# google/deepvariant

Measured on AMD Instinct MI355X. Metric: candidate pileups/sec (encode+CNN), higher is better.
Workload: dtype u8 (encoder) / f16 MFMA, f32 accumulate (CNN); 1 GPU; configs[1] shape: synthetic 30x Illumina pileups, WGS 100x221x7, HIP encode + Inception-v3 MFMA on 1 MI355X per rank, random-init weights; parallelism=interval shards x1, all-gather of probs, collective_world_size=1

## Files before the change

deepvariant_amd/csrc/conv_mfma.h:

```cpp
#ifndef DV_CONV_MFMA_H_
#define DV_CONV_MFMA_H_

#include "conv_common.h"

namespace dv {
namespace convk {

constexpr int kSlabChunks = 8;

inline size_t resident_lds_bytes(const ConvArgs& a) {
  return static_cast<size_t>(a.n_slabs) * kSlabChunks * 3 * 32 * kChunk * 2;
}

void launch_conv(const ConvArgs& a, int nb, hipStream_t stream);
void launch_conv_resident(const ConvArgs& a, int n_cus, hipStream_t stream);
void launch_conv_pool_resident(const ConvArgs& a, int n_cus, hipStream_t stream);
void launch_conv_pool1x1(const ConvArgs& a, int nb, hipStream_t stream);

}
}

#endif
```

deepvariant_amd/csrc/conv_mfma.hip:

```cpp
#include <algorithm>
#include <cstdlib>
#include <type_traits>

#include "conv_mfma.h"

using namespace dv::convk;

namespace {

constexpr int prefetch_depth(int , int ) { return 4; }

struct ChunkWalk {
  int kh, kw;
  unsigned tap_off;
  unsigned chunk_off;
  __device__ __forceinline__ unsigned off() const { return chunk_off + tap_off; }
  __device__ __forceinline__ void advance(const ConvArgs& p) {
    const bool row_end = ++kw == p.KW;
    kw = row_end ? 0 : kw;
    tap_off += row_end ? static_cast<unsigned>((p.ig.wp - p.KW + 1) * 16) : 16u;
    kh += row_end ? 1 : 0;
    const bool taps_end = kh == p.KH;
    kh = taps_end ? 0 : kh;
    tap_off = taps_end ? 0u : tap_off;
// ... 314 lines not shown
  DV_STORE_SLAB(0)
  __syncthreads();

  const int frag_off = (lane >> 5) * (BN * 8) + (lane & 31) * 8;
  if (wave_blank) {
    const int n_full_b = p.n_chunks / SLAB;
    for (int s = 0; s < n_full_b; ++s) {
      const int next = s + 1 < (p.n_chunks + SLAB - 1) / SLAB ? s + 1 : s;
      DV_LOAD_SLAB(next)
      DV_STORE_SLAB((s + 1) & 1)
      __syncthreads();
    }
    copy_blank_wave<NB, PT>(p, n_tile, pn, poh, pow_, mvalid, lane);
    return;
  }
  SidePool<PT> side;
  auto k_loop = [&](auto split_tag, auto pool_tag, const int n_chunks) {
    constexpr bool S = decltype(split_tag)::value;
    constexpr bool P = decltype(pool_tag)::value;
    SidePool<PT>* const sp = P ? &side : nullptr;
    const int tile_slabs = (n_chunks + SLAB - 1) / SLAB;
#ifdef DV_ABLATE_LOOP
    const int n_full = n_chunks < 0 ? 1 : 0;
    const int rem = 0;
#else
    const int n_full = n_chunks / SLAB;
    const int rem = n_chunks - n_full * SLAB;
#endif
    for (int s = 0; s < n_full; ++s) {
      const int next = s + 1 < tile_slabs ? s + 1 : s;
      DV_LOAD_SLAB(next)
      if constexpr (WIDE) {
        conv_slab_wide<NB, PT, SLAB>(p, rsrc, smem + (s & 1) * SLAB_HALFS + frag_off, walk, base, xf, acc);
      } else {
        conv_slab<NB, PT, SLAB, 0, S, P>(p, rsrc, smem + (s & 1) * SLAB_HALFS + frag_off, walk, base, xf, acc, sp);
      }
      DV_STORE_SLAB((s + 1) & 1)
      __syncthreads();
    }
    if (rem) {
      const _Float16* wslab = smem + (n_full & 1) * SLAB_HALFS + frag_off;
      if constexpr (WIDE) {
        conv_slab_wide<NB, PT, 4>(p, rsrc, wslab, walk, base, xf, acc);
        if constexpr (SLAB > 4) {
          if (rem > 4) conv_slab_wide<NB, PT, 4>(p, rsrc, wslab + 4 * BN * kChunk, walk, base, xf, acc);
        }
      } else {
      conv_slab<NB, PT, 4, 0, S, P>(p, rsrc, wslab, walk, base, xf, acc, sp);
      if constexpr (SLAB > 4) {
        if (rem > 4) conv_slab<NB, PT, 4, 4, S, P>(p, rsrc, wslab + 4 * BN * kChunk, walk, base, xf, acc, sp);
      }
      }
    }
  };
  if constexpr (SPLIT) {
    if (n_tile < p.split_tiles) {
      k_loop(std::true_type{}, std::false_type{}, p.n_chunks);
    } else {
      k_loop(std::false_type{}, std::false_type{}, p.n_chunks >> 1);
    }
  } else if constexpr (SIDE_POOL) {
    side.tap = 0;
    side.cc = 0;
    side.cc_mod = 0;
    side.n_tiles = p.n_tiles;
    side.my_tile = n_tile;
    side.taps = p.KH * p.KW;
    side.n_cc = p.Cin / kChunk;
    side.gstride2 = 2u * static_cast<unsigned>(p.side_pool_og.hp * p.side_pool_og.wp);
    side.out = reinterpret_cast<uint4_t*>(p.side_pool_out);
#pragma unroll
    for (int pt = 0; pt < PT; ++pt) {
      const _Float16 lowest = static_cast<_Float16>(-65504.f);
      side.best[pt] = half8_t{lowest, lowest, lowest, lowest, lowest, lowest, lowest, lowest};
      side.ok[pt] = mvalid[pt];
      side.at[pt] = static_cast<unsigned>(
          ((pn[pt] * p.side_pool_og.groups + p.side_pool_goff + (lane >> 5)) * p.side_pool_og.hp + poh[pt] +
           p.side_pool_og.halo) * p.side_pool_og.wp + pow_[pt] + p.side_pool_og.halo);
    }
    k_loop(std::false_type{}, std::true_type{}, p.n_chunks);
  } else {
    k_loop(std::false_type{}, std::false_type{}, p.n_chunks);
  }
#undef DV_LOAD_SLAB
#undef DV_STORE_SLAB

  if constexpr (AVG) {
    conv_epilogue_avg<NB, PT>(acc, p, n_tile, pix_block, pn, poh, pow_, mvalid, lane, wave, smem);
  } else {
    conv_epilogue<NB, PT>(acc, p, n_tile, pn, poh, pow_, mvalid, lane);
  }
}

template <int NB, int PT>
__global__ __launch_bounds__(512, 1) void conv_resident_kernel(ConvArgs p) {
  constexpr int BN = NB * 32;
  constexpr int WAVES = 8, kThreads = WAVES * 64;
  constexpr int SLAB_HALFS = kSlabChunks * BN * kChunk;
  constexpr int kPrefetch = prefetch_depth(NB, PT);
  extern __shared__ __attribute__((aligned(16))) _Float16 smem[];
  const int tid = threadIdx.x, lane = tid & 63, wave = tid >> 6;
  const int blk = blockIdx.x;
  const int n_tile = (blk >> 3) % p.n_tiles;
  const int seq = (blk & 7) + 8 * ((blk >> 3) / p.n_tiles);
  const int n_seq = 8 * ((static_cast<int>(gridDim.x) >> 3) / p.n_tiles);
  {
    const uint4_t* wsrc = reinterpret_cast<const uint4_t*>(p.w) +
                          static_cast<size_t>(n_tile) * p.n_slabs * (kSlabChunks * BN * 2);
    uint4_t* wdst = reinterpret_cast<uint4_t*>(smem);
    const int pieces = p.n_slabs * (kSlabChunks * BN * 2);
    for (int i = tid; i < pieces; i += kThreads) wdst[i] = wsrc[i];
  }
  __syncthreads();
  const int frag_off = (lane >> 5) * (BN * 8) + (lane & 31) * 8;
  const int ohow = p.OH * p.OW;
  const int n_full = p.n_chunks / kSlabChunks;
  const int rem = p.n_chunks - n_full * kSlabChunks;
  const int n_wave_tiles = (p.M + 32 * PT - 1) / (32 * PT);
  for (int wt = seq * WAVES + wave; wt < n_wave_tiles; wt += n_seq * WAVES) {
    int n0 = 0;
    unsigned base[PT];
    int pn[PT], poh[PT], pow_[PT];
    bool mvalid[PT];
#pragma unroll
    for (int pt = 0; pt < PT; ++pt) {
      const int m = (wt * PT + pt) * 32 + (lane & 31);
      int n, pix, oh, ow;
      mvalid[pt] = m < p.M;
      divmod_small(mvalid[pt] ? m : 0, ohow, p.rcp_ohow, n, pix);
      divmod_small(pix, p.OW, p.rcp_ow, oh, ow);
      const int iy = oh * p.stride - p.pad_h + p.ig.halo;
      const int ix = ow * p.stride - p.pad_w + p.ig.halo;
      if (pt == 0) n0 = __builtin_amdgcn_readfirstlane(n);
      base[pt] = mvalid[pt]
                     ? static_cast<unsigned>(((((n - n0) * p.ig.groups + (lane >> 5)) * p.ig.hp + iy) *
                                                  p.ig.wp + ix) * 16)
                     : 0x80000000u;
      pn[pt] = n;
      poh[pt] = oh;
      pow_[pt] = ow;
    }
    const size_t in_off = static_cast<size_t>(n0) * p.img_bytes;
    const size_t in_left = p.in_bytes - in_off;
    const __amdgpu_buffer_rsrc_t rsrc = __builtin_amdgcn_make_buffer_rsrc(
        const_cast<char*>(reinterpret_cast<const char*>(p.in) + in_off), 0,
        static_cast<unsigned>(in_left < 0x7fffffffu ? in_left : 0x7fffffffu), 0x00020000);
    uint4_t xf[kPrefetch][PT];
    float16_t acc[NB][PT];
#pragma unroll
    for (int nb = 0; nb < NB; ++nb)
#pragma unroll
      for (int pt = 0; pt < PT; ++pt)
#pragma unroll
        for (int i = 0; i < 16; ++i) acc[nb][pt][i] = 0.f;
    ChunkWalk walk{0, 0, 0u, 0u};
#pragma unroll
    for (int d = 0; d < kPrefetch; ++d) {
      const unsigned soff = walk.off();
#pragma unroll
      for (int pt = 0; pt < PT; ++pt) {
        xf[d][pt] = __builtin_amdgcn_raw_buffer_load_b128(rsrc, base[pt], soff, 0);
      }
      walk.advance(p);
    }
    for (int s = 0; s < n_full; ++s) {
      conv_slab<NB, PT, kSlabChunks>(p, rsrc, smem + s * SLAB_HALFS + frag_off, walk, base, xf, acc);
    }
    if (rem) {
      const _Float16* wslab = smem + n_full * SLAB_HALFS + frag_off;
      conv_slab<NB, PT, 4>(p, rsrc, wslab, walk, base, xf, acc);
      if (rem > 4) conv_slab<NB, PT, 4, 4>(p, rsrc, wslab + 4 * BN * kChunk, walk, base, xf, acc);
    }
    conv_epilogue<NB, PT>(acc, p, n_tile, pn, poh, pow_, mvalid, lane);
  }
}
// ... 384 lines not shown
  if constexpr (NB >= 3 && NB <= 4) {
    if (slab4 && blocks2 >= 512) {
      hipLaunchKernelGGL((conv_mfma_kernel<NB, 2, 2, 4>), dim3(static_cast<unsigned>(blocks2)),
                         dim3(kConvThreads), static_cast<size_t>(2) * 4 * NB * 32 * kChunk * 2, stream, a);
      return;
    }
    if (w8 && blocks2 >= 1024) {
      hipLaunchKernelGGL((conv_mfma_kernel<NB, 2, 1, kSlabChunks, 8>), dim3(static_cast<unsigned>(blocks(512))),
                         dim3(512), conv_lds_bytes<NB>(), stream, a);
      return;
    }
  }
  if (force_pt ? force_pt == 2 : blocks2 >= 512) {
    if constexpr (NB == 4) {
      static const bool two = getenv("DV_CONV42_BLOCKS") == nullptr || atoi(getenv("DV_CONV42_BLOCKS")) != 1;
      if (two) {
        hipLaunchKernelGGL((conv_mfma_kernel<NB, 2, 2>), dim3(static_cast<unsigned>(blocks2)),
                           dim3(kConvThreads), conv_lds_bytes<NB>(), stream, a);
        return;
      }
    }
    hipLaunchKernelGGL((conv_mfma_kernel<NB, 2>), dim3(static_cast<unsigned>(blocks2)),
                       dim3(kConvThreads), conv_lds_bytes<NB>(), stream, a);
  } else {
    hipLaunchKernelGGL((conv_mfma_kernel<NB, 1>), dim3(static_cast<unsigned>(blocks(128))),
                       dim3(kConvThreads), conv_lds_bytes<NB>(), stream, a);
  }
}

}
namespace dv {
namespace convk {


template <typename K>
static void allow_big_lds(K kernel) {
  (void)hipFuncSetAttribute(reinterpret_cast<const void*>(kernel), hipFuncAttributeMaxDynamicSharedMemorySize, 160 * 1024);
}

void launch_conv_pool_resident(const ConvArgs& a, int n_cus, hipStream_t stream) {
  static const bool attr = (allow_big_lds(conv_pool_resident_kernel<3>), true);
  (void)attr;
  const long frags = (static_cast<long>(a.N) * a.OW + 29) / 30;
  const int per_set = 8 * a.n_tiles;
  const long want = (frags + 8 * 8 - 1) / (8 * 8) * per_set;
  const int grid = static_cast<int>(std::max<long>(per_set, std::min<long>(want, n_cus / per_set * per_set)));
  hipLaunchKernelGGL((conv_pool_resident_kernel<3>), dim3(grid), dim3(512), resident_lds_bytes(a), stream, a);
}

void launch_conv_pool1x1(const ConvArgs& a, int nb, hipStream_t stream) {
  const size_t lds = static_cast<size_t>(a.n_slabs) * kSlabChunks * nb * 32 * kChunk * 2;
  const dim3 grid(static_cast<unsigned>(((a.M + 127) / 128) * a.n_tiles));
  switch (nb) {
    case 7: {
      static const bool attr = (allow_big_lds(conv_pool1x1_kernel<7, 8>), true);
      (void)attr;
      hipLaunchKernelGGL((conv_pool1x1_kernel<7, 8>), dim3(static_cast<unsigned>((a.M + 255) / 256)), dim3(512), lds, stream, a);
      break;
    }
    case 1: hipLaunchKernelGGL((conv_pool1x1_kernel<1>), grid, dim3(kConvThreads), lds, stream, a); break;
    case 2: hipLaunchKernelGGL((conv_pool1x1_kernel<2>), grid, dim3(kConvThreads), lds, stream, a); break;
    case 3: hipLaunchKernelGGL((conv_pool1x1_kernel<3>), grid, dim3(kConvThreads), lds, stream, a); break;
    default: hipLaunchKernelGGL((conv_pool1x1_kernel<4>), grid, dim3(kConvThreads), lds, stream, a); break;
  }
}

void launch_conv_resident(const ConvArgs& a, int n_cus, hipStream_t stream) {
  static const bool attr = (allow_big_lds(conv_resident_kernel<3, 2>), true);
  (void)attr;
  const int grid = n_cus / (8 * a.n_tiles) * (8 * a.n_tiles);
  hipLaunchKernelGGL((conv_resident_kernel<3, 2>), dim3(grid), dim3(512), resident_lds_bytes(a), stream, a);
}

void launch_conv(const ConvArgs& a, int nb, hipStream_t stream) {
  switch (nb) {
    case 1: ::launch_conv<1>(a, stream); break;
    case 2: ::launch_conv<2>(a, stream); break;
    case 3: ::launch_conv<3>(a, stream); break;
    case 6: launch_conv6(a, stream); break;
    default: ::launch_conv<4>(a, stream); break;
  }
}

}
}
```

deepvariant_amd/csrc/model.hip:

```cpp
#include <algorithm>
#include <map>
#include <atomic>
#include <cmath>
#include <cstdlib>
#include <cstring>
#include <memory>
#include <thread>

#include <hip/hip_fp16.h>

#include "model_graph.h"
#include "model_kernels.h"
#include "block35.h"
#include "chain.h"
#include "stem_fused.h"
#include "calib.h"
#include "layer_export.h"

namespace {

static int stem_sub_batch() {
  static const int v = getenv("DV_STEM_SB") ? std::max(1, atoi(getenv("DV_STEM_SB"))) : (1 << 30);
  return v;
}
// ... 296 lines not shown
  a.w = op.ow;
  a.n_tiles = (n + a.G - 1) / a.G;
  a.n_layers = op.chain_len;
  double tr_flops = 0;
  std::string tr_label = "chain";
  size_t act = 0, slot = 0;
  for (int k = 0; k < op.chain_len; ++k) {
    const Op& o = m->ops[oi + k];
    dv::ChainLayer& cl = a.L[k];
    cl.w = m->w_ptr(o);
    cl.shift = m->shift_ptr(o);
    cl.n_chunks = o.cin / kChunk;
    cl.cout = o.cout;
    cl.cout_pad = (o.cout + 31) / 32 * 32;
    cl.kh = o.kh;
    cl.kw = o.kw;
    cl.slab_bytes = static_cast<unsigned>(o.kh * o.kw * 2 * cl.cout_pad * 16);
    act = std::max(act, static_cast<size_t>(o.cin / 8) * op.chain_tpx * 16);
    slot = std::max(slot, static_cast<size_t>(cl.slab_bytes));
    tr_flops += 2.0 * n * o.oh * o.ow * o.kh * o.kw * o.cin * o.cout;
    tr_label += " " + std::to_string(o.kh) + "x" + std::to_string(o.kw) + ":" + std::to_string(o.cin) + "->" +
                std::to_string(o.cout);
  }
  a.act_bytes = static_cast<unsigned>(act);
  a.slot_bytes = static_cast<unsigned>(slot);
  a.out = m->buf_ptr(last.out_buf);
  a.og = m->buffers[last.out_buf].geom();
  a.out_goff = last.out_coff / 8;
  tr_label += " @" + std::to_string(op.oh) + "x" + std::to_string(op.ow) + " [fused, G=" + std::to_string(a.G) + "]";
  TraceScope tr(ps.stream, tr_label, tr_flops,
                2.0 * n * op.oh * op.ow * (static_cast<double>(op.cin) + last.cout));
  dv::ProfileScope prof(dv::kProfConv, ps.stream);
  static const bool chain_prof = getenv("DV_CHAIN_PROF") != nullptr;
  if (chain_prof && g_trace != nullptr) {
    report_chain_profile(a, m->n_cus, ps.stream);
  } else {
    dv::launch_chain(a, m->n_cus, ps.stream);
  }
  return op.chain_len;
}

int enqueue_first_conv(const Pass& ps, int oi) {
  const dv_model* m = ps.m;
  const int n = ps.n;
  const Op& op = m->ops[oi];
  FirstConvArgs f{};
  f.ext = ext_table(m);
  f.in_off = ps.images_off;
  f.w = m->w_ptr(op);
  f.shift = m->shift_ptr(op);
  f.out = ps.out_ptr(op.out_buf);
  f.og = m->buffers[op.out_buf].geom();
  f.N = n;
  f.H = op.ih;
  f.W = op.iw;
  f.C = op.cin_real;
  f.Cout = op.cout;
  f.OH = op.oh;
  f.OW = op.ow;
  f.KH = op.kh;
  f.KW = op.kw;
  f.stride = op.stride;
  f.M = n * op.oh * op.ow;
  f.n_chunks = op.n_chunks;
  f.wide = op.cin_real > 8 ? 1 : 0;
  f.in_bytes = static_cast<unsigned>(static_cast<size_t>(n) * op.ih * op.iw * op.cin_real);
  f.rcp_ow = 1.0f / static_cast<float>(op.ow);
  f.rcp_ohow = 1.0f / static_cast<float>(op.oh * op.ow);
  TraceScope tr(ps.stream, "conv_first_u8 3x3 s2 " + std::to_string(op.cin_real) + "->" + std::to_string(op.cout),
                2.0 * f.M * op.kh * op.kw * op.cin_real * op.cout,
                static_cast<double>(n) * (op.ih * op.iw * op.cin_real + 2.0 * op.oh * op.ow * op.cout));
  dv::ProfileScope prof(dv::kProfConv, ps.stream);
  launch_conv_first_u8(f, ps.stream);
  return 1;
}

void set_branch_output(const Pass& ps, const Op& o, ConvBranch& br) {
  const BufferDesc& b = ps.m->buffers[o.out_buf];
  br.out = ps.out_ptr(o.out_buf);
  br.out32 = b.f32 ? ps.m->buf_ptr<float>(o.out_buf) : nullptr;
  br.og = b.geom();
  br.lo_groups = b.wide ? b.c / 8 : 0;
  br.out_goff = o.out_coff / 8;
}

int enqueue_conv(Pass& ps, int oi) {
  const dv_model* m = ps.m;
  const int n = ps.n;
  const Op& op = m->ops[oi];
  ConvArgs a{};
  a.in = m->buf_ptr(op.in_buf);
  const BufferDesc& ib = m->buffers[op.in_buf];
  a.ig = ib.geom();
  a.N = n;
  a.Cin = op.cin;
  a.OH = op.oh;
  a.OW = op.ow;
  static const int cu_pair = getenv("DV_CU_PAIR") ? atoi(getenv("DV_CU_PAIR")) : 0;
  a.cu_pair = cu_pair;
  a.band = op.band;
  a.KH = op.band ? op.band : op.kh;
  a.KW = op.kw;
  a.stride = op.stride;
  a.pad_h = op.pad_h;
  a.pad_w = op.pad_w;
  a.chunk_stride = static_cast<unsigned>(2 * a.ig.hp * a.ig.wp * 16);
  a.M = n * op.oh * op.ow;
  a.n_chunks = op.n_chunks;
  a.n_slabs = op.n_steps;
  a.split = op.split ? 1 : 0;
  a.split_tiles = op.split_tiles;
  a.wide_in = op.in_wide ? 1 : 0;
  a.lo_off = op.in_wide ? static_cast<unsigned>(ib.c / 8) * static_cast<unsigned>(a.ig.hp * a.ig.wp) * 16u : 0u;
  a.in_bytes = static_cast<size_t>(n) * ib.bytes_per_example();
  a.img_bytes = static_cast<unsigned>(ib.bytes_per_example());
  a.rcp_ow = 1.0f / static_cast<float>(op.ow);
  a.rcp_ohow = 1.0f / static_cast<float>(op.oh * op.ow);
  int subs = 0;
  a.n_branches = 0;
  double tr_flops = 0, tr_bytes = static_cast<double>(n) * op.ih * op.iw * op.cin * 2.0;
  std::string tr_label = "conv " + std::to_string(op.kh) + "x" + std::to_string(op.kw) + " s" +
                         std::to_string(op.stride) + " " + std::to_string(op.cin) + "->";
  for (int gi = 0; gi <= op.group_followers; ++gi) {
    const Op& bo = m->ops[oi + gi];
    tr_flops += 2.0 * n * op.oh * op.ow * op.kh * op.kw * op.cin_real * bo.cout;
    tr_bytes += 2.0 * n * op.oh * op.ow * bo.cout;
    tr_label += (gi ? "+" : "") + std::to_string(bo.cout);
    ConvBranch& br = a.br[a.n_branches++];
    br.shift = bo.raw ? nullptr : m->shift_ptr(bo);
    set_branch_output(ps, bo, br);
    br.Cout = bo.cout;
    br.relu = bo.raw ? 0 : 1;
    br.sub0 = subs;
    subs += (bo.cout + 31) / 32;
    if (op.avg_tile_g > 0 && bo.avg_partner >= 0 && bo.avg_partner < ps.last) {
      const Op& pl = m->ops[bo.avg_partner];
      br.avgpool = 1;
      br.shift = m->shift_ptr(pl);
      br.relu = 1;
      set_branch_output(ps, pl, br);
      a.tile_g = op.avg_tile_g;
      a.tile_p = op.oh * op.ow;
      a.rcp_tile_p = 1.0f / static_cast<float>(a.tile_p);
    }
  }
  if (a.tile_g > 0) tr_label += " [+ avgpool3s1 in the epilogue, " + std::to_string(a.tile_g) + " maps per block]";
  a.w = m->w_ptr(op);
  const int tiles = (subs + op.nb - 1) / op.nb;
  a.n_tiles = tiles;
  if (m->blank_on() && m->blank_conv4_op >= 0 && &op == &m->ops[m->blank_conv4_op] &&
      a.n_branches == 1 && !op.band && !op.v2 && !op.pool_in) {
    a.blank_row = m->blank_thr(op.pool_out ? 4 : 3);
    a.blank_src = static_cast<const _Float16*>(m->d_blank_conv4.ptr);
    tr_label += " [blank rows copied]";
  }
  if (m->blank_on() && oi == 1 && !m->ops[0].stem_a && a.n_branches == 1 && !op.band && !op.v2 && !op.pool_in &&
      !op.pool_out && !op.split && op.nb <= 4 && m->d_blank_c2.ptr != nullptr) {
    a.blank_row = m->blank_thr(1);
    a.blank_src = static_cast<const _Float16*>(m->d_blank_c2.ptr);
    if (m->ops[2].stem_b) a.blank_need = m->blank_thr(5);
    tr_label += " [blank rows copied]";
  }
  const int oi_last = oi + op.group_followers;
  tr_label += " @" + std::to_string(op.oh) + "x" + std::to_string(op.ow) + " nb" + std::to_string(op.nb) +
              " tiles" + std::to_string(tiles);
  if (op.pool_in) tr_label += " <- maxpool3s2";
  if (op.in_wide) tr_label += " [hi+lo input: 2 MFMAs per weight fragment]";
  if (op.v2) tr_label += " [imgconv G=" + std::to_string(op.v2_g) + "]";
  if (op.band) tr_label += " [band: " + std::to_string(op.band) + " of " + std::to_string(op.kh) + " tap rows]";
  if (op.split) tr_label += " [split W: " + std::to_string(op.split_tiles) + " of " + std::to_string(tiles) + " tiles]";
  if (op.side_pool_partner > oi_last && op.side_pool_partner < ps.last && op.nb == 4 && !resident_ok(m, op, a)) {
    const Op& pl = m->ops[op.side_pool_partner];
    a.side_pool_out = m->buf_ptr(pl.out_buf);
    a.side_pool_og = m->buffers[pl.out_buf].geom();
    a.side_pool_goff = pl.out_coff / 8;
    ps.side_pooled[op.side_pool_partner] = 1;
    tr_label += " + maxpool3s2 on the side";
    tr_bytes += 2.0 * n * pl.oh * pl.ow * pl.cin;
  }
  const bool resident = !op.v2 && !op.pool_in && !op.pool_out && resident_ok(m, op, a);
  if (resident) tr_label += " [weights resident in LDS]";
  if (op.pool_out) tr_label += " [weights resident in LDS] -> maxpool3s2";
  TraceScope tr(ps.stream, tr_label, tr_flops, tr_bytes);
  dv::ProfileScope prof(dv::kProfConv, ps.stream);
  if (op.pool_out) {
    launch_conv_pool_resident(a, m->n_cus, ps.stream);
  } else if (op.v2) {
    dv::ImgConvArgs ia = m->imgconv_geometry(op, op.v2_g);
    ia.c = a;
    ia.n_img_tiles = (n + op.v2_g - 1) / op.v2_g;
    ia.n_cout_tiles = op.v2_tiles;
    dv::launch_imgconv(ia, op.nb, m->n_cus, ps.stream);
  } else if (op.pool_in) {
    a.stride = 2;
    launch_conv_pool1x1(a, op.nb, ps.stream);
  } else if (resident) {
    launch_conv_resident(a, m->n_cus, ps.stream);
  } else {
    launch_conv(a, op.nb, ps.stream);
  }
  return op.group_followers + 1;
}

int enqueue_pool(const Pass& ps, int oi) {
  const dv_model* m = ps.m;
  const int n = ps.n;
  const Op& op = m->ops[oi];
  const BufferDesc &ib = m->buffers[op.in_buf], &ob = m->buffers[op.out_buf];
  PoolArgs p{};
  p.in = m->buf_ptr(op.in_buf);
  p.in32 = m->buf_ptr<float>(op.in_buf);
  p.out = ps.out_ptr(op.out_buf);
  p.out32 = ob.f32 ? m->buf_ptr<float>(op.out_buf) : nullptr;
  p.lo_in_groups = ib.wide ? ib.c / 8 : 0;
  p.lo_out_groups = ob.wide ? ob.c / 8 : 0;
  p.ig = ib.geom();
  p.og = ob.geom();
  p.N = n;
  p.C = op.cin;
  p.OH = op.oh;
  p.OW = op.ow;
  p.out_goff = op.out_coff / 8;
  p.shift = op.pool_shift_relu ? m->shift_ptr(op) : nullptr;
  TraceScope tr(ps.stream, std::string(op.type == kOpMaxPool ? "maxpool3s2 " : "avgpool3s1 ") +
                               std::to_string(op.cin) + " @" + std::to_string(op.oh) + "x" + std::to_string(op.ow),
                0.0, 2.0 * n * op.cin * (static_cast<double>(op.ih) * op.iw + op.oh * op.ow));
  dv::ProfileScope prof(dv::kProfOther, ps.stream);
  if (op.type == kOpMaxPool) {
    if (ib.f32 || ob.f32) return dv::fail(DV_ERR_UNSUPPORTED, "max-pool of a float32 tensor");
    launch_maxpool3s2(p, ps.stream);
  } else {
    if (!ib.f32) return dv::fail(DV_ERR_UNSUPPORTED, "average pool of an fp16 tensor");
    launch_avgpool3s1(p, ps.stream);
  }
  return 1;
}

int run_ops(dv_model* m, int first, int last, int n, hipStream_t stream,
            int shifted_buf = -1, int out_example_off = 0, size_t images_off = 0) {
  Pass ps{m, n, stream, first, last, shifted_buf, out_example_off, images_off, std::vector<char>(m->ops.size(), 0)};
  for (int oi = first; oi < last;) {
    const Op& op = m->ops[oi];
    int ran = 1;
    if (ps.side_pooled[oi]) {
    } else if (op.type == kOpAvgPool && op.avg_partner >= 0 && m->ops[op.avg_partner].avg_partner == oi &&
               op.avg_partner >= first) {
    } else if (op.type != kOpConv) {
      ran = enqueue_pool(ps, oi);
    } else if (op.stem_a) {
      ran = enqueue_stem_a(ps, oi);
    } else if (op.stem_b) {
      ran = enqueue_stem_b(ps, oi);
    } else if (op.b35 == 1) {
      ran = enqueue_block35(ps, oi);
    } else if (op.chain_len > 0) {
      ran = enqueue_chain(ps, oi);
    } else if (op.first_u8) {
      ran = enqueue_first_conv(ps, oi);
    } else {
      ran = enqueue_conv(ps, oi);
    }
    if (ran < 0) return ran;
    oi += ran;
  }
  DV_HIP_CHECK(hipGetLastError());
  return DV_OK;
}

}

extern "C" {

int dv_model_create(const dv_model_desc* desc, int device, dv_model** out) {
  if (!desc || !out) return dv::fail(DV_ERR_INVALID_ARGUMENT, "dv_model_create: null");
  if (desc->channels < 1 || desc->channels > 16 || desc->num_classes < 1 ||
      desc->num_classes > 8 || desc->max_batch < 1 || desc->max_batch > 8192 ||
      desc->height < 75 ||
      desc->width < 75) {
    return dv::fail(DV_ERR_INVALID_ARGUMENT,
                    "dv_model_create: unsupported shape (need H,W >= 75, C <= 16, max_batch <= 8192)");
// ... 361 lines not shown
      c.keep_f32 = m->buffers[op.out_buf].f32 || m->buffers[op.out_buf].wide ? 1 : 0;
      if (op.pool_in) {
        plan.bufs[op.in_buf].h = op.ih;
        plan.bufs[op.in_buf].w = op.iw;
      }
      if (op.pool_out) {
        oh = (oh - 3) / 2 + 1;
        ow = (ow - 3) / 2 + 1;
      }
    } else if (op.type == kOpAvgPool) {
      c.shift_relu = op.pool_shift_relu;
      if (op.pool_shift_relu) c.shift_off = static_cast<int64_t>(op.shift_off);
      c.cout = op.cout;
      c.keep_f32 = m->buffers[op.out_buf].f32 || m->buffers[op.out_buf].wide ? 1 : 0;
    } else {
      c.cout = op.cout;
    }
    plan.bufs[op.out_buf].h = oh;
    plan.bufs[op.out_buf].w = ow;
    plan.ops.push_back(c);
  }
  plan.feat_buf = m->feat_buf;
  plan.num_classes = m->desc.num_classes;
  plan.dense_off = m->layers.back().param_off;
  return plan;
}

int dv_model_calibrate(dv_model* m, const float* weights, int64_t n_weights, const uint8_t* images, int n_images,
                       float* corrections, int64_t capacity) {
  if (!m || !weights || !images) return dv::fail(DV_ERR_INVALID_ARGUMENT, "dv_model_calibrate: null");
  if (!m->loaded) return dv::fail(DV_ERR_INVALID_ARGUMENT, "dv_model_calibrate: load weights first");
  if (n_weights != m->n_params) return dv::fail(DV_ERR_INVALID_ARGUMENT, "dv_model_calibrate: wrong number of weights");
  if (n_images < 1 || n_images > 4096) return dv::fail(DV_ERR_INVALID_ARGUMENT, "dv_model_calibrate: 1..4096 images");
  const dv::CalibPlan plan = calib_plan_of(m);
  std::vector<float> corr, dense_corr;
  if (int rc = dv::run_calibration(plan, m->device, weights, n_weights, m->h_shift, images, n_images, &corr,
                                   &dense_corr)) {
    return rc;
  }
  std::vector<float> shift = m->h_shift, dense_b = m->h_dense_b;
  for (size_t i = 0; i < shift.size(); ++i) shift[i] -= corr[i];
  for (size_t k = 0; k < dense_b.size(); ++k) dense_b[k] -= dense_corr[k];
  DV_HIP_CHECK(hipSetDevice(m->device));
  DV_HIP_CHECK(hipDeviceSynchronize());
  DV_HIP_CHECK(hipMemcpy(m->d_shift.ptr, shift.data(), shift.size() * 4, hipMemcpyHostToDevice));
  DV_HIP_CHECK(hipMemcpy(m->d_dense_b.ptr, dense_b.data(), dense_b.size() * 4, hipMemcpyHostToDevice));
  if (corrections != nullptr) {
    int64_t at = 0;
    for (size_t off : m->correction_shift_offsets()) {
      if (at < capacity) corrections[at++] = corr[off];
    }
    for (size_t k = 0; k < dense_corr.size() && at < capacity; ++k) corrections[at++] = dense_corr[k];
  }
  return prepare_blank_responses(m);
}

int dv_model_apply_corrections(dv_model* m, const float* corrections, int64_t n) {
  if (!m || !corrections) return dv::fail(DV_ERR_INVALID_ARGUMENT, "dv_model_apply_corrections: null");
  if (!m->loaded) return dv::fail(DV_ERR_INVALID_ARGUMENT, "dv_model_apply_corrections: load weights first");
  const std::vector<size_t> offs = m->correction_shift_offsets();
  if (n != static_cast<int64_t>(offs.size() + m->h_dense_b.size())) return dv::fail(DV_ERR_INVALID_ARGUMENT, "dv_model_apply_corrections: wrong number of corrections");
  for (int64_t i = 0; i < n; ++i) {
    if (!std::isfinite(corrections[i])) return dv::fail(DV_ERR_BAD_INPUT, "dv_model_apply_corrections: non-finite correction");
  }
  std::vector<float> shift = m->h_shift, dense_b = m->h_dense_b;
  int64_t at = 0;
  for (size_t off : offs) shift[off] -= corrections[at++];
  for (size_t k = 0; k < dense_b.size(); ++k) dense_b[k] -= corrections[at++];
  DV_HIP_CHECK(hipSetDevice(m->device));
  DV_HIP_CHECK(hipDeviceSynchronize());
  DV_HIP_CHECK(hipMemcpy(m->d_shift.ptr, shift.data(), shift.size() * 4, hipMemcpyHostToDevice));
  DV_HIP_CHECK(hipMemcpy(m->d_dense_b.ptr, dense_b.data(), dense_b.size() * 4, hipMemcpyHostToDevice));
  return prepare_blank_responses(m);
}

int dv_model_num_ops(const dv_model* m) { return m ? static_cast<int>(m->ops.size()) : 0; }

int dv_model_op_label(const dv_model* m, int op_index, char* buf, int capacity) {
  if (!m || !buf || capacity < 1 || op_index < 0 || op_index >= static_cast<int>(m->ops.size())) {
    return dv::fail(DV_ERR_INVALID_ARGUMENT, "dv_model_op_label: bad argument");
  }
  const Op& op = m->ops[op_index];
  const char* kind = op.type == kOpConv ? "conv" : op.type == kOpMaxPool ? "maxpool" : "avgpool";
  snprintf(buf, static_cast<size_t>(capacity), "%s layer=%d k=%dx%d s=%d cin=%d cout=%d out=%dx%d raw=%d in_buf=%d out_buf=%d coff=%d lds_only=%d",
           kind, op.layer, op.kh, op.kw, op.stride, op.cin, op.cout, op.oh, op.ow, op.raw ? 1 : 0, op.in_buf, op.out_buf,
           op.out_coff, (op.type == kOpConv && (op.stem_a || op.stem_b)) || (op_index + 1 < static_cast<int>(m->ops.size()) && m->ops[op_index + 1].in_chain && m->ops[op_index + 1].in_buf == op.out_buf) ||
               (op.b35 >= 2 && op.b35 <= 4) || op.b35 == 6 ? 1 : 0);
  return DV_OK;
}

int dv_model_probe_rounding(dv_model* m, const float* weights, int64_t n_weights, const uint8_t* images, int n_images,
                            const uint8_t* keep_f32, int flags, const float* corrections, int64_t n_corrections,
                            float* logits_r, float* logits_e, float* corrections_out) {
  if (!m || !weights || !images || !logits_e) return dv::fail(DV_ERR_INVALID_ARGUMENT, "dv_model_probe_rounding: null");
  if (!m->loaded) return dv::fail(DV_ERR_INVALID_ARGUMENT, "dv_model_probe_rounding: load weights first");
  if (n_weights != m->n_params) return dv::fail(DV_ERR_INVALID_ARGUMENT, "dv_model_probe_rounding: wrong number of weights");
  if (n_images < 1 || n_images > 4096) return dv::fail(DV_ERR_INVALID_ARGUMENT, "dv_model_probe_rounding: 1..4096 images");
  dv::CalibPlan plan = calib_plan_of(m);
  if (keep_f32 != nullptr) {
    for (size_t i = 0; i < plan.ops.size(); ++i) plan.ops[i].keep_f32 = keep_f32[i] ? 1 : 0;
  }
  std::vector<float> corr_in(m->h_shift.size(), 0.f), dense_in(m->h_dense_b.size(), 0.f);
  if (corrections != nullptr) {
    const std::vector<size_t> offs = m->correction_shift_offsets();
    if (n_corrections != static_cast<int64_t>(offs.size() + dense_in.size())) return dv::fail(DV_ERR_INVALID_ARGUMENT, "dv_model_probe_rounding: wrong number of corrections");
    int64_t at = 0;
    for (size_t off : offs) corr_in[off] = corrections[at++];
    for (size_t k = 0; k < dense_in.size(); ++k) dense_in[k] = corrections[at++];
  }
  const bool measure = (flags & 2) != 0;
  if (measure && corrections != nullptr) return dv::fail(DV_ERR_INVALID_ARGUMENT, "dv_model_probe_rounding: measure or apply");
  dv::CalibProbe probe;
  probe.corr_in = measure ? nullptr : corr_in.data();
  probe.dense_corr_in = measure ? nullptr : dense_in.data();
  probe.logits_r = logits_r;
  probe.logits_e = logits_e;
  probe.skip_r = logits_r == nullptr && !measure;
  probe.weights_f32 = (flags & 1) != 0;
  std::vector<float> corr, dense_corr;
  if (int rc = dv::run_calibration(plan, m->device, weights, n_weights, m->h_shift, images, n_images, &corr, &dense_corr,
                                   &probe)) {
    return rc;
  }
  if (corrections_out != nullptr) {
    int64_t at = 0;
    for (size_t off : m->correction_shift_offsets()) corrections_out[at++] = corr[off];
    for (float v : dense_corr) corrections_out[at++] = v;
  }
  return DV_OK;
}

int dv_model_debug_tensor(dv_model* m, int index, int n, void* host_out, int32_t* h,
                          int32_t* w, int32_t* c) {
  if (m && index == -1) index = m->feat_buf;
  if (m && index == -2) index = m->stem_out_buf;
  if (!m || index < 0 || index >= static_cast<int>(m->buffers.size())) {
    return dv::fail(DV_ERR_INVALID_ARGUMENT, "dv_model_debug_tensor: bad index");
  }
  const BufferDesc& b = m->buffers[index];
  if (h) *h = b.h + 2 * b.halo;
  if (w) *w = b.w + 2 * b.halo;
  if (c) *c = b.c;
  if (host_out) {
    DV_HIP_CHECK(hipSetDevice(m->device));
    DV_HIP_CHECK(hipDeviceSynchronize());
    if (b.f32) {
      std::vector<float> tmp(static_cast<size_t>(n) * b.bytes_per_example() / 4);
      DV_HIP_CHECK(hipMemcpy(tmp.data(), m->dbuf[index].ptr, tmp.size() * 4, hipMemcpyDeviceToHost));
      _Float16* dst = static_cast<_Float16*>(host_out);
      for (size_t i = 0; i < tmp.size(); ++i) dst[i] = static_cast<_Float16>(tmp[i]);
    } else if (b.wide) {
      const size_t half_halfs = b.bytes_per_example() / 4;
      std::vector<_Float16> tmp(static_cast<size_t>(n) * half_halfs * 2);
      DV_HIP_CHECK(hipMemcpy(tmp.data(), m->dbuf[index].ptr, tmp.size() * 2, hipMemcpyDeviceToHost));
      _Float16* dst = static_cast<_Float16*>(host_out);
      for (int e = 0; e < n; ++e)
        for (size_t i = 0; i < half_halfs; ++i) {
          dst[static_cast<size_t>(e) * half_halfs + i] = static_cast<_Float16>(
              static_cast<float>(tmp[static_cast<size_t>(e) * 2 * half_halfs + i]) +
              static_cast<float>(tmp[static_cast<size_t>(e) * 2 * half_halfs + half_halfs + i]));
        }
    } else {
      DV_HIP_CHECK(hipMemcpy(host_out, m->dbuf[index].ptr,
                             static_cast<size_t>(n) * b.bytes_per_example(),
                             hipMemcpyDeviceToHost));
    }
  }
  return DV_OK;
}

// ... 241 lines not shown
```

deepvariant_amd/csrc/model_graph.cpp:

```cpp
#include <algorithm>
#include <cstdlib>

#include "model_graph.h"
#include "model_kernels.h"
#include "block35.h"
#include "chain.h"
#include "stem_fused.h"

int dv_model::new_buffer(int h, int w, int c) {
  buffers.push_back({h, w, c, 0});
  buffers.back().wide = precise && wide_stage;
  return static_cast<int>(buffers.size()) - 1;
}
int dv_model::pick_nb(int cout) {
  static const bool nb6 = getenv("DV_NB6") != nullptr && atoi(getenv("DV_NB6")) != 0;
  if (nb6 && cout > 128 && cout <= 192) return 6;
  int best = 4, best_cost = 1 << 30, best_waste = 1 << 30;
  for (int nb = 4; nb >= 1; --nb) {
    const int bn = nb * 32;
    const int tiles = (cout + bn - 1) / bn;
    const int cost = tiles * (nb + 1), waste = tiles * bn - cout;
    if (cost < best_cost || (cost == best_cost && waste < best_waste)) {
      best_cost = cost;
      best_waste = waste;
// ... 502 lines not shown
    const int oh = (x.h - 3) / 2 + 1, ow = (x.w - 3) / 2 + 1;
    const int out = new_buffer(oh, ow, 384 + 96 + x.c);
    conv(x, 384, 3, 3, 2, false, out, 0);
    TensorRef b = conv(x, 64, 1, 1);
    b = conv(b, 96, 3, 3);
    conv(b, 96, 3, 3, 2, false, out, 384);
    pool(kOpMaxPool, x, out, 480);
    named_views.push_back({"mixed3", out, 0, buffers[out].c});
    x = full(out);
  }
  wide_stage = true;
  for (int c7 : {128, 160, 160, 192}) {
    const int out = new_buffer(x.h, x.w, 768);
    conv(x, 192, 1, 1, 1, true, out, 0);
    TensorRef b = conv(x, c7, 1, 1);
    b = conv(b, c7, 1, 7);
    conv(b, 192, 7, 1, 1, true, out, 192);
    TensorRef d = conv(x, c7, 1, 1);
    d = conv(d, c7, 7, 1);
    d = conv(d, c7, 1, 7);
    d = conv(d, c7, 7, 1);
    conv(d, 192, 1, 7, 1, true, out, 384);
    pooled_projection(x, 192, out, 576);
    named_views.push_back({"mixed" + std::to_string(named_views.size()), out, 0, buffers[out].c});
    x = full(out);
  }
  {
    const int oh = (x.h - 3) / 2 + 1, ow = (x.w - 3) / 2 + 1;
    const int out = new_buffer(oh, ow, 320 + 192 + x.c);
    TensorRef b = conv(x, 192, 1, 1);
    conv(b, 320, 3, 3, 2, false, out, 0);
    TensorRef d = conv(x, 192, 1, 1);
    d = conv(d, 192, 1, 7);
    d = conv(d, 192, 7, 1);
    conv(d, 192, 3, 3, 2, false, out, 320);
    pool(kOpMaxPool, x, out, 512);
    named_views.push_back({"mixed8", out, 0, buffers[out].c});
    x = full(out);
  }
  for (int i = 0; i < 2; ++i) {
    const int out = new_buffer(x.h, x.w, 2048);
    conv(x, 320, 1, 1, 1, true, out, 0);
    TensorRef b = conv(x, 384, 1, 1);
    conv(b, 384, 1, 3, 1, true, out, 320);
    conv(b, 384, 3, 1, 1, true, out, 704);
    named_views.push_back({"mixed9_" + std::to_string(i), out, 320, 2 * 384});
    TensorRef d = conv(x, 448, 1, 1);
    d = conv(d, 384, 3, 3);
    conv(d, 384, 1, 3, 1, true, out, 1088);
    conv(d, 384, 3, 1, 1, true, out, 1472);
    pooled_projection(x, 192, out, 1856);
    named_views.push_back({"mixed" + std::to_string(9 + i), out, 0, buffers[out].c});
    x = full(out);
  }
  feat_buf = x.buf;
  buffers[feat_buf].f32 = true;
  buffers[feat_buf].wide = false;
  feat_p = x.h * x.w;
  feat_c = x.c;
  group_siblings();
  for (const Op& op : ops) {
    int need = 0;
    if (op.type == kOpConv) need = std::max(op.pad_h, op.pad_w);
    if (op.type == kOpAvgPool) need = 1;
    buffers[op.in_buf].halo = std::max(buffers[op.in_buf].halo, need);
  }
  choose_chains();
  if (getenv("DV_CHAIN_KEEP_HALO") == nullptr) {
    for (BufferDesc& b : buffers) b.halo = 0;
    for (const Op& op : ops) {
      if (op.in_chain) continue;
      int need = 0;
      if (op.type == kOpConv && op.chain_len == 0) need = std::max(op.pad_h, op.pad_w);
      if (op.type == kOpAvgPool) need = 1;
      buffers[op.in_buf].halo = std::max(buffers[op.in_buf].halo, need);
    }
  }
  choose_imgconv();
  choose_band();
  choose_split();
  choose_side_pool();
  choose_avg_epilogue();
  choose_block35();
  for (size_t i = 0; i < ops.size(); ++i) {
    Op& op = ops[i];
    if (op.type != kOpConv) continue;
    int subs = 0;
    for (int gi = 0; gi <= op.group_followers; ++gi) subs += (ops[i + gi].cout + 31) / 32;
    const int n_tiles = (subs + op.nb - 1) / op.nb;
    for (int gi = 0; gi <= op.group_followers; ++gi) ops[i + gi].w_off = packed_halfs;
    packed_halfs += op.first_u8 ? static_cast<size_t>(kFirstMaxChunks) * 32 * kChunk
                    : op.b35 == 1 ? static_cast<size_t>(2) * (op.cin / kChunk) * 2 * 128 * 8
                    : (op.chain_len > 0 || op.in_chain || op.b35 >= 5)
                        ? static_cast<size_t>(op.n_chunks) * 2 * ((op.cout + 31) / 32 * 32) * 8
                    : op.v2     ? static_cast<size_t>(op.v2_tiles) * op.v2_steps *
                                      dv::imgconv_wslab_halfs(op.kh, op.kw, op.nb)
                                : static_cast<size_t>(op.band ? op.band : 1) * n_tiles * op.n_steps *
                                      kSlabChunks * (op.nb * 32) * kChunk;
    i += op.group_followers;
  }
  layers.push_back({1, 1, feat_c, desc.num_classes, n_params});
  n_params += static_cast<int64_t>(feat_c) * desc.num_classes + desc.num_classes;
}

std::vector<size_t> dv_model::correction_shift_offsets() const {
  std::vector<const Op*> by_layer(layers.size(), nullptr);
  for (const Op& op : ops) {
    if (op.type == kOpConv) by_layer[op.layer] = &op;
  }
  std::vector<size_t> at;
  for (size_t l = 0; l + 1 < layers.size(); ++l) {
    for (int co = 0; co < by_layer[l]->cout; ++co) at.push_back(by_layer[l]->shift_off + co);
  }
  return at;
}
```

deepvariant_amd/csrc/model_graph.h:

```cpp
#ifndef DV_MODEL_GRAPH_H_
#define DV_MODEL_GRAPH_H_

#include <string>
#include <vector>

#include "dv_internal.h"
#include "conv_mfma.h"
#include "imgconv.h"

namespace dv {
namespace graph {

using namespace convk;

struct TensorRef {
  int buf = -1;
  int h = 0, w = 0, c = 0;
};

struct BufferDesc {
  int h, w, c;
  int halo = 0;
  int min_examples = 1;
  bool f32 = false;
  bool wide = false;
  TensorGeom geom() const {
    return TensorGeom{h, w, halo, h + 2 * halo, w + 2 * halo, (wide ? 2 : 1) * (c / 8)};
  }
  size_t bytes_per_example() const {
    return static_cast<size_t>(h + 2 * halo) * (w + 2 * halo) * c * (f32 ? 4 : wide ? 4 : 2);
  }
};

enum OpType { kOpConv, kOpMaxPool, kOpAvgPool };

struct Op {
  OpType type;
  int in_buf, out_buf;
  int out_coff = 0;
  int layer = -1;
  int kh = 0, kw = 0, stride = 1, pad_h = 0, pad_w = 0;
  int cin = 0, cin_real = 0, cout = 0;
  bool in_wide = false;
  int ih = 0, iw = 0, oh = 0, ow = 0;
  int nb = 4;
  int n_steps = 0, n_chunks = 0;
  size_t w_off = 0;
  size_t shift_off = 0;
  size_t tbl_off = 0;
  bool raw = false;
  int group_followers = 0;
  bool first_u8 = false;
  bool pool_shift_relu = false;
  bool pool_in = false;
  int side_pool_partner = -1;
  int avg_partner = -1;
  int avg_tile_g = 0;
  bool pool_out = false;
  int band = 0;
  bool split = false;
  bool split_rows = false;
  int split_tiles = 0;
  bool v2 = false;
  int v2_g = 0;
  int v2_steps = 0;
  int v2_tiles = 0;
  bool stem_a = false;
  bool stem_b = false;
  int chain_len = 0;
  int chain_g = 0;
  int chain_tpx = 0;
  bool in_chain = false;
  int b35 = 0;
};

struct LayerInfo {
  int kh, kw, cin, cout;
  int64_t param_off;
};

}
}

using namespace dv::graph;

struct dv_model {
  int device = 0;
  dv_model_desc desc{};
  std::vector<BufferDesc> buffers;
  std::vector<Op> ops;
  std::vector<LayerInfo> layers;
  int64_t n_params = 0;
  int feat_buf = -1, feat_p = 0, feat_c = 0;
  int stem_ops_end = 0, stem_out_buf = -1;
  int stem_a_grid = 512, stem_b_grid = 256;
  int n_cus = 256;
  size_t packed_halfs = 0, shift_floats = 0, tbl_entries = 0;
  std::vector<dv::DeviceBuffer> dbuf;
  dv::DeviceBuffer d_w, d_shift, d_dense_w, d_dense_b, d_tbl;
  bool blank_skip = false;
  bool blank_enabled = true;
  bool blank_ready = false;
  int blank_conv4_op = -1;
  dv::DeviceBuffer d_blank_thr;
  dv::DeviceBuffer d_blank_conv4;
  dv::DeviceBuffer d_blank_c2;
  dv::DeviceBuffer d_blank_b;
  bool blank_on() const { return blank_ready && blank_enabled; }
  bool precise = false;
  bool wide_stage = false;
  bool loaded = false;
  std::vector<float> h_shift, h_dense_b;
  dv::DeviceBuffer d_ext;
  struct GraphEntry {
    int n;
    hipStream_t stream;
    hipGraphExec_t exec;
  };
  std::vector<GraphEntry> graphs;
  int64_t graph_captures = 0, graph_replays = 0;
  struct NamedView {
    std::string name;
    int buf, coff, c;
  };
  std::vector<NamedView> named_views;

  template <typename T = _Float16>
  T* buf_ptr(int buf) const { return static_cast<T*>(dbuf[buf].ptr); }
  const _Float16* w_ptr(const Op& op) const { return static_cast<const _Float16*>(d_w.ptr) + op.w_off; }
  const float* shift_ptr(const Op& op) const { return static_cast<const float*>(d_shift.ptr) + op.shift_off; }
  const int* blank_thr(int row) const { return static_cast<const int*>(d_blank_thr.ptr) + row * desc.max_batch; }

  int new_buffer(int h, int w, int c);
  static int pick_nb(int cout);
  TensorRef conv(TensorRef x, int cout, int kh, int kw, int stride = 1, bool same = true,
                 int dst_buf = -1, int dst_coff = 0, int cin_real = -1);
  TensorRef full(int buf) const;
  void pooled_projection(TensorRef x, int cout, int dst_buf, int dst_coff);
  TensorRef pool(OpType type, TensorRef x, int dst_buf = -1, int dst_coff = 0);
  void group_siblings();
  dv::ImgConvArgs imgconv_geometry(const Op& op, int g) const;
  void choose_imgconv();
  void choose_band();
  void choose_side_pool();
  void choose_split();
  void choose_avg_epilogue();
  void choose_chains();
  void choose_block35();
  void build();
  std::vector<size_t> correction_shift_offsets() const;
};

#endif
```

Measured before the change: 520,100 candidates/s.

## Add persistent conv kernel overlapping next item's prefetch with current epilogue

```diff
diff --git a/deepvariant_amd/csrc/conv_mfma.h b/deepvariant_amd/csrc/conv_mfma.h
--- a/deepvariant_amd/csrc/conv_mfma.h
+++ b/deepvariant_amd/csrc/conv_mfma.h
@@ -16,6 +16,9 @@
 void launch_conv_resident(const ConvArgs& a, int n_cus, hipStream_t stream);
 void launch_conv_pool_resident(const ConvArgs& a, int n_cus, hipStream_t stream);
 void launch_conv_pool1x1(const ConvArgs& a, int nb, hipStream_t stream);
+bool conv_heads_ok(const ConvArgs& a, int nb);
+int conv_heads_grid(const ConvArgs& a, int n_cus);
+void launch_conv_heads(const ConvArgs& a, int n_cus, hipStream_t stream, unsigned long long* prof);
 
 }
 }
diff --git a/deepvariant_amd/csrc/conv_mfma.hip b/deepvariant_amd/csrc/conv_mfma.hip
--- a/deepvariant_amd/csrc/conv_mfma.hip
+++ b/deepvariant_amd/csrc/conv_mfma.hip
@@ -420,8 +420,6 @@
   } else {
     k_loop(std::false_type{}, std::false_type{}, p.n_chunks);
   }
-#undef DV_LOAD_SLAB
-#undef DV_STORE_SLAB
 
   if constexpr (AVG) {
     conv_epilogue_avg<NB, PT>(acc, p, n_tile, pix_block, pn, poh, pow_, mvalid, lane, wave, smem);
@@ -429,6 +427,241 @@
     conv_epilogue<NB, PT>(acc, p, n_tile, pn, poh, pow_, mvalid, lane);
   }
 }
+
+struct HeadsProf {
+  unsigned long long first_slab = 0;
+  unsigned long long k_loop = 0;
+  unsigned long long epi = 0;
+  unsigned long long epi_avg = 0;
+  unsigned long long change = 0;
+  unsigned long long setup = 0;
+  unsigned long long items = 0;
+};
+__device__ __forceinline__ unsigned long long heads_clock() { return __builtin_amdgcn_s_memtime(); }
+
+struct HeadsItem {
+  int n_tile, pix_block;
+  int n0;
+  unsigned base[2];
+  int pn[2], poh[2], pow_[2];
+  bool mvalid[2];
+};
+
+template <bool AVG, bool PROF = false>
+__global__ __launch_bounds__(256, 2) void conv_heads_kernel(ConvArgs p, int n_items, unsigned long long* prof_out) {
+  constexpr int NB = 4, PT = 2, SLAB = kSlabChunks, WAVES = 4;
+  constexpr int BN = NB * 32;
+  constexpr int kThreads = WAVES * 64;
+  constexpr int SLAB_HALFS = SLAB * BN * kChunk;
+  constexpr int SLAB_PIECES = SLAB_HALFS / 8;
+  constexpr int W_PER_THREAD = SLAB_PIECES / kThreads;
+  constexpr int kPrefetch = prefetch_depth(NB, PT);
+  extern __shared__ __attribute__((aligned(16))) _Float16 smem[];
+  HeadsProf prof;
+  unsigned long long t0 = 0;
+  if (PROF) t0 = heads_clock();
+
+  const int tid = threadIdx.x;
+  const int lane = tid & 63;
+  const int wave = tid >> 6;
+  const int xq = n_items >> 3, xr = n_items & 7;
+  const int xcd = blockIdx.x & 7;
+  const int grid = gridDim.x;
+  const int slots = (grid >> 3) + (xcd < (grid & 7) ? 1 : 0);
+  const int cnt = xcd < xr ? xq + 1 : xq;
+  const int first = xcd < xr ? xcd * (xq + 1) : xr * (xq + 1) + (xcd - xr) * xq;
+  int xi = blockIdx.x >> 3;
+  if (xi >= cnt) return;
+
+  const int ohow = p.OH * p.OW;
+  auto locate = [&](int logical, bool live, HeadsItem& it) {
+    int lane_now = lane;
+    asm volatile("" : "+v"(lane_now));
+    it.n_tile = logical % p.n_tiles;
+    it.pix_block = logical / p.n_tiles;
+    const int m_block = it.pix_block * (32 * PT * WAVES);
+    it.n0 = 0;
+#pragma unroll
+    for (int pt = 0; pt < PT; ++pt) {
+      int n, pix, oh, ow;
+      if constexpr (AVG) {
+        int il;
+        divmod_small((wave * PT + pt) * 32 + (lane_now & 31), p.tile_p, p.rcp_tile_p, il, pix);
+        n = it.pix_block * p.tile_g + il;
+        it.mvalid[pt] = live && il < p.tile_g && n < p.N;
+        n = min(n, p.N - 1);
+      } else {
+        const int m = m_block + (wave * PT + pt) * 32 + (lane_now & 31);
+        const bool in_range = m < p.M;
+        it.mvalid[pt] = live && in_range;
+        divmod_small(in_range ? m : 0, ohow, p.rcp_ohow, n, pix);
+      }
+      divmod_small(pix, p.OW, p.rcp_ow, oh, ow);
+      const int iy = oh * p.stride - p.pad_h + p.ig.halo;
+      const int ix = ow * p.stride - p.pad_w + p.ig.halo;
+      const unsigned rel = static_cast<unsigned>((((lane_now >> 5) * p.ig.hp + iy) * p.ig.wp + ix) * 16);
+      if (pt == 0) it.n0 = __builtin_amdgcn_readfirstlane(n);
+      it.base[pt] = it.mvalid[pt] ? static_cast<unsigned>(n - it.n0) * p.img_bytes + rel
+                                  : 0x80000000u;
+      it.pn[pt] = n;
+      it.poh[pt] = oh;
+      it.pow_[pt] = ow;
+    }
+  };
+  auto descriptor = [&](int n0) {
+    const size_t in_off = static_cast<size_t>(n0) * p.img_bytes;
+    const size_t in_left = p.in_bytes - in_off;
+    return __builtin_amdgcn_make_buffer_rsrc(const_cast<char*>(reinterpret_cast<const char*>(p.in) + in_off), 0,
+                                             static_cast<unsigned>(in_left < 0x7fffffffu ? in_left : 0x7fffffffu),
+                                             0x00020000);
+  };
+  const size_t tile_pieces = static_cast<size_t>(p.n_slabs) * (kSlabChunks * BN * 2);
+  auto pooled_tile = [&](int n_tile) {
+    bool any = false;
+#pragma unroll
+    for (int nb = 0; nb < NB; ++nb) {
+      const int sub = n_tile * NB + nb;
+      const ConvBranch& b = p.br[branch_of(p, sub)];
+      any = any || ((sub - b.sub0) * 32 < b.Cout && b.avgpool != 0);
+    }
+    return any;
+  };
+
+  const int frag_off = (lane >> 5) * (BN * 8) + (lane & 31) * 8;
+  const int n_full = p.n_chunks / SLAB;
+  const int rem = p.n_chunks - n_full * SLAB;
+  const int tile_slabs = n_full + (rem ? 1 : 0);
+
+  unsigned base[PT];
+  __amdgpu_buffer_rsrc_t rsrc;
+  const uint4* wtile;
+  {
+    HeadsItem it;
+    locate(first + xi, true, it);
+#pragma unroll
+    for (int pt = 0; pt < PT; ++pt) base[pt] = it.base[pt];
+    rsrc = descriptor(it.n0);
+    wtile = reinterpret_cast<const uint4*>(p.w) + static_cast<size_t>(it.n_tile) * tile_pieces;
+  }
+  const uint4* wsrc = wtile;
+  uint4_t wreg[W_PER_THREAD];
+  uint4_t xf[kPrefetch][PT];
+  float16_t acc[NB][PT];
+  ChunkWalk walk{0, 0, 0u, 0u};
+  DV_LOAD_SLAB(0)
+#pragma unroll
+  for (int d = 0; d < kPrefetch; ++d) {
+    const unsigned soff = walk.off();
+#pragma unroll
+    for (int pt = 0; pt < PT; ++pt) xf[d][pt] = __builtin_amdgcn_raw_buffer_load_b128(rsrc, base[pt], soff, 0);
+    walk.advance(p);
+  }
+  DV_STORE_SLAB(0)
+  __syncthreads();
+  int buf0 = 0;
+  if (PROF) {
+    const unsigned long long t = heads_clock();
+    prof.setup += t - t0;
+    t0 = t;
+  }
+
+  for (;;) {
+    const int xi_next = xi + slots;
+    const bool more = xi_next < cnt;
+    const int logical_next = first + (more ? xi_next : xi);
+    const uint4* wtile_next = more ? reinterpret_cast<const uint4*>(p.w) + static_cast<size_t>(logical_next % p.n_tiles) * tile_pieces
+                                   : wtile + static_cast<size_t>(tile_slabs - 1) * SLAB_PIECES;
+#pragma unroll
+    for (int nb = 0; nb < NB; ++nb)
+#pragma unroll
+      for (int pt = 0; pt < PT; ++pt)
+#pragma unroll
+        for (int i = 0; i < 16; ++i) acc[nb][pt][i] = 0.f;
+    for (int s = 0; s < n_full; ++s) {
+      wsrc = s + 1 < tile_slabs ? wtile + static_cast<size_t>(s + 1) * SLAB_PIECES : wtile_next;
+      DV_LOAD_SLAB(0)
+      conv_slab<NB, PT, SLAB>(p, rsrc, smem + ((buf0 + s) & 1) * SLAB_HALFS + frag_off, walk, base, xf, acc);
+      DV_STORE_SLAB((buf0 + s + 1) & 1)
+      __syncthreads();
+      if (PROF && s == 0) prof.first_slab += heads_clock() - t0;
+    }
+    if (rem) {
+      const _Float16* wslab = smem + ((buf0 + n_full) & 1) * SLAB_HALFS + frag_off;
+      wsrc = wtile_next;
+      DV_LOAD_SLAB(0)
+      conv_slab<NB, PT, 4>(p, rsrc, wslab, walk, base, xf, acc);
+      if (rem > 4) conv_slab<NB, PT, 4, 4>(p, rsrc, wslab + 4 * BN * kChunk, walk, base, xf, acc);
+      DV_STORE_SLAB((buf0 + n_full + 1) & 1)
+      __syncthreads();
+    }
+    buf0 = (buf0 + tile_slabs) & 1;
+    if (PROF) {
+      const unsigned long long t = heads_clock();
+      prof.k_loop += t - t0;
+      prof.items += 1;
+      t0 = t;
+    }
+
+    HeadsItem nxt;
+    locate(logical_next, more, nxt);
+    const __amdgpu_buffer_rsrc_t rsrc_next = descriptor(nxt.n0);
+    walk = ChunkWalk{0, 0, 0u, 0u};
+#pragma unroll
+    for (int d = 0; d < kPrefetch; ++d) {
+      const unsigned soff = walk.off();
+#pragma unroll
+      for (int pt = 0; pt < PT; ++pt) xf[d][pt] = __builtin_amdgcn_raw_buffer_load_b128(rsrc_next, nxt.base[pt], soff, 0);
+      walk.advance(p);
+    }
+
+    HeadsItem cur;
+    locate(first + xi, true, cur);
+    bool pooled = false;
+    if constexpr (AVG) {
+      pooled = pooled_tile(cur.n_tile);
+      int lane_now = lane;
+      asm volatile("" : "+v"(lane_now));
+      conv_epilogue_avg<NB, PT>(acc, p, cur.n_tile, cur.pix_block, cur.pn, cur.poh, cur.pow_, cur.mvalid, lane_now, wave, smem);
+    } else {
+      conv_epilogue<NB, PT>(acc, p, cur.n_tile, cur.pn, cur.poh, cur.pow_, cur.mvalid, lane);
+    }
+    if (PROF) {
+      const unsigned long long t = heads_clock();
+      (pooled ? prof.epi_avg : prof.epi) += t - t0;
+      t0 = t;
+    }
+    if (!more) break;
+    if (pooled) {
+      wsrc = wtile_next;
+      DV_LOAD_SLAB(0)
+      __syncthreads();
+      DV_STORE_SLAB(buf0)
+      __syncthreads();
+      if (PROF) {
+        const unsigned long long t = heads_clock();
+        prof.change += t - t0;
+        t0 = t;
+      }
+    }
+#pragma unroll
+    for (int pt = 0; pt < PT; ++pt) base[pt] = nxt.base[pt];
+    rsrc = rsrc_next;
+    wtile = wtile_next;
+    xi = xi_next;
+  }
+  if (PROF && lane == 0 && prof_out != nullptr) {
+    unsigned long long* dst = prof_out + (static_cast<size_t>(blockIdx.x) * WAVES + wave) * 8;
+    dst[0] = prof.first_slab;
+    dst[1] = prof.k_loop;
+    dst[2] = prof.epi;
+    dst[3] = prof.epi_avg;
+    dst[4] = prof.change;
+    dst[5] = prof.setup;
+    dst[6] = prof.items;
+  }
+}
+#undef DV_LOAD_SLAB
+#undef DV_STORE_SLAB
 
 template <int NB, int PT>
 __global__ __launch_bounds__(512, 1) void conv_resident_kernel(ConvArgs p) {
@@ -979,5 +1212,34 @@
   }
 }
 
-}
-}
+bool conv_heads_ok(const ConvArgs& a, int nb) {
+  if (nb != 4 || a.split || a.wide_in || a.side_pool_out != nullptr || a.band || a.blank_row != nullptr || a.cu_pair) return false;
+  if (a.tile_g > 0) return true;
+  if (getenv("DV_CONV_PT") || getenv("DV_CONV_SLAB4") || getenv("DV_CONV_W8") || getenv("DV_CONV42_BLOCKS")) return false;
+  return (static_cast<long>(a.M) + 255) / 256 * a.n_tiles >= 512;
+}
+
+int conv_heads_grid(const ConvArgs& a, int n_cus) {
+  const long blocks = a.tile_g > 0 ? (static_cast<long>(a.N) + a.tile_g - 1) / a.tile_g : (static_cast<long>(a.M) + 255) / 256;
+  return static_cast<int>(std::min<long>(blocks * a.n_tiles, 2L * n_cus));
+}
+
+void launch_conv_heads(const ConvArgs& a, int n_cus, hipStream_t stream, unsigned long long* prof) {
+  const long blocks = a.tile_g > 0 ? (static_cast<long>(a.N) + a.tile_g - 1) / a.tile_g : (static_cast<long>(a.M) + 255) / 256;
+  const int items = static_cast<int>(blocks * a.n_tiles);
+  const dim3 grid(static_cast<unsigned>(conv_heads_grid(a, n_cus)));
+  if (a.tile_g > 0) {
+    if (prof != nullptr) {
+      hipLaunchKernelGGL((conv_heads_kernel<true, true>), grid, dim3(kConvThreads), conv_lds_bytes<4>(), stream, a, items, prof);
+    } else {
+      hipLaunchKernelGGL((conv_heads_kernel<true>), grid, dim3(kConvThreads), conv_lds_bytes<4>(), stream, a, items, prof);
+    }
+  } else if (prof != nullptr) {
+    hipLaunchKernelGGL((conv_heads_kernel<false, true>), grid, dim3(kConvThreads), conv_lds_bytes<4>(), stream, a, items, prof);
+  } else {
+    hipLaunchKernelGGL((conv_heads_kernel<false>), grid, dim3(kConvThreads), conv_lds_bytes<4>(), stream, a, items, prof);
+  }
+}
+
+}
+}
diff --git a/deepvariant_amd/csrc/model.hip b/deepvariant_amd/csrc/model.hip
--- a/deepvariant_amd/csrc/model.hip
+++ b/deepvariant_amd/csrc/model.hip
@@ -402,6 +402,27 @@
   br.og = b.geom();
   br.lo_groups = b.wide ? b.c / 8 : 0;
   br.out_goff = o.out_coff / 8;
+}
+
+void report_heads_profile(const ConvArgs& a, int n_cus, hipStream_t stream) {
+  const int grid = conv_heads_grid(a, n_cus);
+  const size_t words = static_cast<size_t>(grid) * 4 * 8;
+  unsigned long long* d = nullptr;
+  if (hipMalloc(&d, words * 8) != hipSuccess) return;
+  (void)hipMemsetAsync(d, 0, words * 8, stream);
+  launch_conv_heads(a, n_cus, stream, d);
+  std::vector<unsigned long long> h(words);
+  (void)hipStreamSynchronize(stream);
+  (void)hipMemcpy(h.data(), d, words * 8, hipMemcpyDeviceToHost);
+  (void)hipFree(d);
+  double sum[7] = {0, 0, 0, 0, 0, 0, 0};
+  for (size_t w = 0; w < static_cast<size_t>(grid) * 4; ++w)
+    for (int i = 0; i < 7; ++i) sum[i] += static_cast<double>(h[w * 8 + i]);
+  const double items = std::max(sum[6], 1.0), waves = static_cast<double>(grid) * 4;
+  fprintf(stderr, "[dv-heads] %d workgroups, %.1f items per wave; cycles per item and wave: first slab %.0f, K loop %.0f "
+                  "(%d slabs), plain epilogue %.0f, pooling epilogue %.0f, slab 0 back after pooling %.0f; set-up %.0f per wave\n",
+          grid, items / waves, sum[0] / items, sum[1] / items, a.n_slabs, sum[2] / items, sum[3] / items, sum[4] / items,
+          sum[5] / waves);
 }
 
 int enqueue_conv(Pass& ps, int oi) {
@@ -500,6 +521,9 @@
   }
   const bool resident = !op.v2 && !op.pool_in && !op.pool_out && resident_ok(m, op, a);
   if (resident) tr_label += " [weights resident in LDS]";
+  const bool heads = !op.pool_out && !op.v2 && !op.pool_in && !resident && m->persistent_heads && conv_heads_ok(a, op.nb);
+  if (heads) tr_label += " [persistent]";
+  ps.m->ops[oi].heads_launch = heads;
   if (op.pool_out) tr_label += " [weights resident in LDS] -> maxpool3s2";
   TraceScope tr(ps.stream, tr_label, tr_flops, tr_bytes);
   dv::ProfileScope prof(dv::kProfConv, ps.stream);
@@ -516,6 +540,13 @@
     launch_conv_pool1x1(a, op.nb, ps.stream);
   } else if (resident) {
     launch_conv_resident(a, m->n_cus, ps.stream);
+  } else if (heads) {
+    static const bool heads_prof = getenv("DV_HEADS_PROF") != nullptr;
+    if (heads_prof && g_trace != nullptr) {
+      report_heads_profile(a, m->n_cus, ps.stream);
+    } else {
+      launch_conv_heads(a, m->n_cus, ps.stream, nullptr);
+    }
   } else {
     launch_conv(a, op.nb, ps.stream);
   }
@@ -1043,10 +1074,10 @@
   }
   const Op& op = m->ops[op_index];
   const char* kind = op.type == kOpConv ? "conv" : op.type == kOpMaxPool ? "maxpool" : "avgpool";
-  snprintf(buf, static_cast<size_t>(capacity), "%s layer=%d k=%dx%d s=%d cin=%d cout=%d out=%dx%d raw=%d in_buf=%d out_buf=%d coff=%d lds_only=%d",
+  snprintf(buf, static_cast<size_t>(capacity), "%s layer=%d k=%dx%d s=%d cin=%d cout=%d out=%dx%d raw=%d in_buf=%d out_buf=%d coff=%d lds_only=%d persistent=%d",
            kind, op.layer, op.kh, op.kw, op.stride, op.cin, op.cout, op.oh, op.ow, op.raw ? 1 : 0, op.in_buf, op.out_buf,
            op.out_coff, (op.type == kOpConv && (op.stem_a || op.stem_b)) || (op_index + 1 < static_cast<int>(m->ops.size()) && m->ops[op_index + 1].in_chain && m->ops[op_index + 1].in_buf == op.out_buf) ||
-               (op.b35 >= 2 && op.b35 <= 4) || op.b35 == 6 ? 1 : 0);
+               (op.b35 >= 2 && op.b35 <= 4) || op.b35 == 6 ? 1 : 0, op.heads_launch ? 1 : 0);
   return DV_OK;
 }
 
diff --git a/deepvariant_amd/csrc/model_graph.cpp b/deepvariant_amd/csrc/model_graph.cpp
--- a/deepvariant_amd/csrc/model_graph.cpp
+++ b/deepvariant_amd/csrc/model_graph.cpp
@@ -608,6 +608,7 @@
   choose_side_pool();
   choose_avg_epilogue();
   choose_block35();
+  persistent_heads = getenv("DV_NO_PERSISTENT_HEADS") == nullptr;
   for (size_t i = 0; i < ops.size(); ++i) {
     Op& op = ops[i];
     if (op.type != kOpConv) continue;
diff --git a/deepvariant_amd/csrc/model_graph.h b/deepvariant_amd/csrc/model_graph.h
--- a/deepvariant_amd/csrc/model_graph.h
+++ b/deepvariant_amd/csrc/model_graph.h
@@ -72,6 +72,7 @@
   int chain_tpx = 0;
   bool in_chain = false;
   int b35 = 0;
+  bool heads_launch = false;
 };
 
 struct LayerInfo {
@@ -108,6 +109,7 @@
   dv::DeviceBuffer d_blank_b;
   bool blank_on() const { return blank_ready && blank_enabled; }
   bool precise = false;
+  bool persistent_heads = true;
   bool wide_stage = false;
   bool loaded = false;
   std::vector<float> h_shift, h_dense_b;
```

Result: no change. 518,100 candidates/s (-0.4%).
